# index-tts/index-tts

Hardware: AMD Instinct MI355X
Metric: audio-seconds/sec (RTF) IndexTTS-2.5, 64-utt batch @1/2/4/8 MI355X (higher is better)
Workload: dtype bf16 (GPT GEMM operands / KV cache; f32 accumulate, residual stream, norms: the reference's own GPU mode) + fp32x3 (flow matching: f32 activations / weights / accumulation, GEMM and attention products on the bf16 matrix pipe with every f32 operand carried exactly as three bf16 planes = 24 significan

## Files before the change

### indextts_amd/csrc/capi_s2mel.hip

```cpp
#include <math.h>
#include <stdlib.h>
#include <string.h>
#include <algorithm>
#include <map>
#include <string>
#include <vector>

#include "../../include/indextts_hip.h"
#include "gpt_kernels.h"
#include "s2mel_kernels.h"

static bool s2_fused(int precision, bool opt_fused) {
    if (precision == PREC_F32X3) return true;
    return (precision == PREC_BF16 || precision == PREC_F32) && opt_fused;
}

struct S2Layer {
    void *w_qkv = 0, *w_o = 0, *w_13 = 0, *w_2 = 0, *w_skip_a = 0, *w_skip_b = 0;
    float *g_attn = 0, *g_ffn = 0, *b_skip = 0;
};
struct S2Wn {
    void *w_in = 0, *w_rs = 0;
    float *b_in = 0, *b_rs = 0;
};

struct itts_s2mel {
    itts_s2mel_config cfg;
    int I = 0, Kx = 0;
    std::map<std::string, std::pair<std::vector<float>, std::vector<int64_t>>> host;
    std::vector<S2Layer> layers;
    std::vector<S2Wn> wn;
    float* g_norm = 0;
    void *w_x = 0, *w_sl_a = 0, *w_sl_b = 0, *w_c1 = 0, *w_rp = 0, *w_fl = 0, *w_c2 = 0;
    float *b_sl = 0, *b_c1 = 0, *b_rp = 0, *b_fl = 0, *b_c2 = 0;
    std::vector<void*> owned;
    bool finalized = false;
    bool opt_fused = true;
// ... 287 lines not shown
        if (!rc) rc = f.pack_kn(Fin::cols_kn(*wc2, C, W, 0, W), W, W, C, &h->w_c2);
        if (!rc) rc = f.vec(bc2, &h->b_c2);
    }
    for (int i = 0; i < L && rc == ITTS_OK; ++i) {
        const std::string a = P + "wavenet.in_layers." + std::to_string(i) + ".conv.conv.", b = P + "wavenet.res_skip_layers." + std::to_string(i) + ".conv.conv.";
        const int ro = i < L - 1 ? 2 * W : W;
        NEED(wi, a + "weight", 2 * W, W, k);
        NEED(bi, a + "bias", 2 * W);
        NEED(wr, b + "weight", ro, W, 1);
        NEED(br, b + "bias", ro);
        if (!wi || !bi || !wr || !br) continue;
        std::vector<float> kn((size_t)k * W * 2 * W);
        for (int n = 0; n < 2 * W; ++n)
            for (int cc = 0; cc < W; ++cc)
                for (int j = 0; j < k; ++j) kn[((size_t)j * W + cc) * 2 * W + n] = (*wi)[((size_t)n * W + cc) * k + j];
        rc = f.pack_kn(f.pair_tiles(kn, k * W, 2 * W), k * W, k * W, 2 * W, &h->wn[i].w_in);
        if (!rc) rc = f.vec(bi, &h->wn[i].b_in);
        if (!rc) rc = f.pack_kn(Fin::cols_kn(*wr, ro, W, 0, W), W, W, ro, &h->wn[i].w_rs);
        if (!rc) rc = f.vec(br, &h->wn[i].b_rs);
    }
#undef NEED
    if (rc) return rc;
    if (!f.missing.empty()) { itts_set_error("s2mel_finalize: missing or mis-shaped tensors: %s", f.missing.c_str()); return ITTS_ERR_STATE; }
    h->host.clear();
    h->finalized = true;
    return ITTS_OK;
}

extern "C" int itts_s2mel_mods_per_step(const itts_s2mel* h) {
    if (!h) return 0;
    const itts_s2mel_config& c = h->cfg;
    return c.depth * 4 * c.hidden_dim + 2 * c.hidden_dim + c.wavenet_layers * 2 * c.wavenet_hidden + 2 * c.wavenet_hidden;
}

static size_t s_a256(size_t x) { return (x + 255) & ~(size_t)255; }

struct S2Ws {
    float *X, *X2, *BIG, *WX, *OUT, *RP, *D;
    char *HB, *QA, *AO, *FC, *COL, *XA, *SK, *KC, *VC, *WXA, *ZR, *HBP;
    size_t hbp_stride;
    size_t sk_stride, total;
};

static S2Ws s2_carve(const itts_s2mel* h, char* base, int n_tok, int n_seq, int t_pad) {
    const itts_s2mel_config& c = h->cfg;
    const size_t N = (size_t)n_tok, H = c.hidden_dim, I = h->I, W = c.wavenet_hidden, C = c.in_channels, Kx = h->Kx;
    const size_t esz = c.precision == PREC_BF16 ? 2 : 4;
    const size_t big = std::max(std::max(3 * H, 2 * I), 2 * W);
    const size_t hw = std::max(H, W), fw = std::max(I, W);
    S2Ws w;
    size_t off = 0;
    auto take = [&](size_t bytes) { char* p = base ? base + off : nullptr; off += s_a256(bytes); return p; };
    w.X = (float*)take(N * H * 4);
    w.X2 = (float*)take(N * H * 4);
    w.BIG = (float*)take(N * big * 4);
    w.WX = (float*)take(N * W * 4);
    w.OUT = (float*)take(N * W * 4);
    w.RP = (float*)take(N * W * 4);
    w.D = (float*)take(N * C * 4);
    w.HB = take(N * hw * esz);
    w.QA = take(N * H * esz);
    w.AO = take(N * H * esz);
    w.FC = take(N * fw * esz);
    w.COL = take(N * (size_t)c.wavenet_kernel * W * esz);
    w.XA = take(N * Kx * esz);
    w.sk_stride = s_a256(N * H * esz);
    w.SK = take(w.sk_stride * (size_t)(c.depth / 2));
    w.WXA = take(N * W * esz);
    w.hbp_stride = (N * H + 127) / 128 * 128;
    w.HBP = take(c.precision == PREC_F32X3 ? w.hbp_stride * 6 : 0);
    const size_t kv = (size_t)n_seq * c.num_heads * t_pad * 64 * (c.precision == PREC_F32X3 ? 6 : esz);
    w.ZR = take(256);
    w.KC = take(kv);
    w.VC = take(kv);
    w.total = off + 256;
    return w;
}

extern "C" size_t itts_s2mel_workspace_bytes(const itts_s2mel* h, int n_tok, int n_seq, int t_max) {
    if (!h || n_tok <= 0 || n_seq <= 0 || t_max <= 0) return 0;
    return s2_carve(h, nullptr, n_tok, n_seq, (t_max + 63) / 64 * 64).total;
}

// ... 117 lines not shown
    const float* m_gc = m_norm + 2 * H;
    const float* m_fl = m_gc + (size_t)c.wavenet_layers * 2 * W;
    const SeqTab& tt = tail ? *tail : tab;
    const void* XAt = w.XA;
    if (tail) {
        if ((rc = launch_cast_pad(x_src, w.QA, tail->n_tok, src_rows, C, Kx, prec, st, tail_src))) return rc;
        XAt = w.QA;
    }
    const int NT = tt.n_tok;
    if ((rc = launch_ada_rmsnorm(X, h->g_norm, m_norm, w.HB, NT, H, c.norm_eps, prec, st, tail && !prune_last ? tail_src : nullptr))) return rc;
    S2_TRACE("final ada_rmsnorm -> HB", w.HB, (size_t)NT * H * esz);
    if ((rc = s2_gemm(h, w.HB, H, h->w_sl_a, h->b_sl, X2, H, NT, H, H, EPI_STORE_F32, st))) return rc;
    if ((rc = s2_gemm(h, XAt, Kx, h->w_sl_b, nullptr, X2, H, NT, H, Kx, EPI_RESIDUAL, st, fused ? w.HB : nullptr))) return rc;
    if (!fused && (rc = launch_cast_pad(X2, w.HB, NT, NT, H, H, prec, st))) return rc;
    S2_TRACE("skip_linear -> X2", X2, (size_t)NT * H * 4);
    if ((rc = s2_gemm(h, w.HB, H, h->w_c1, h->b_c1, w.WX, W, NT, W, H, EPI_STORE_F32, st, fused ? w.WXA : nullptr))) return rc;
    S2_TRACE("conv1 -> WX", w.WX, (size_t)NT * W * 4);
    if ((rc = s2_gemm(h, w.HB, H, h->w_rp, h->b_rp, w.RP, W, NT, W, H, EPI_STORE_F32, st))) return rc;
    int dil = 1;
    for (int i = 0; i < c.wavenet_layers; ++i) {
        const S2Wn& Wn = h->wn[i];
        const int last = i == c.wavenet_layers - 1;
        if (!fused && (rc = launch_im2col_reflect(w.WX, w.COL, tt, W, c.wavenet_kernel, dil, prec, st))) return rc;
        const int ro = last ? W : 2 * W;
        if (fused) {
            GemmArgs g{};
            g.A = w.WXA; g.lda = W; g.Wp = Wn.w_in; g.bias = Wn.b_in; g.M = NT; g.N = 2 * W; g.K = c.wavenet_kernel * W;
            g.nsplit = 1; g.epi = EPI_GATE; g.out_act = w.FC; g.gvec = m_gc + (size_t)i * 2 * W; g.D = W;
            g.conv_taps = c.wavenet_kernel; g.conv_dil = dil; g.conv_W = W; g.tok_seq = tt.tok_seq; g.tok_t = tt.tok_t;
            g.seq_start = tt.seq_start; g.seq_T = tt.seq_T; g.zero_row = w.ZR;
            if ((rc = s2_launch_gemm(h, g, st))) return rc;
            GemmArgs r{};
            r.A = w.FC; r.lda = W; r.Wp = Wn.w_rs; r.bias = Wn.b_rs; r.M = NT; r.N = ro; r.K = W; r.nsplit = 1; r.epi = EPI_WN_RS;
            r.out_f32 = w.WX; r.out2 = w.OUT; r.D = W; r.wn_first = i == 0; r.wn_last = last; r.out_act2 = last ? nullptr : w.WXA;
            r.tok_seq = tt.tok_seq; r.tok_t = tt.tok_t; r.seq_len = tt.seq_len;
            S2_TRACE("wavenet in_layer + gate -> FC", w.FC, (size_t)NT * W * esz);
            if ((rc = s2_launch_gemm(h, r, st))) return rc;
            S2_TRACE("wavenet res_skip -> WX", w.WX, (size_t)NT * W * 4);
            S2_TRACE("wavenet res_skip -> OUT", w.OUT, (size_t)NT * W * 4);
        } else {
            if ((rc = s2_gemm(h, w.COL, c.wavenet_kernel * W, Wn.w_in, Wn.b_in, w.BIG, 2 * W, NT, 2 * W, c.wavenet_kernel * W, EPI_STORE_F32, st))) return rc;
            if ((rc = launch_wn_gate(w.BIG, m_gc + (size_t)i * 2 * W, w.FC, NT, W, prec, st))) return rc;
            if ((rc = s2_gemm(h, w.FC, W, Wn.w_rs, Wn.b_rs, w.BIG, ro, NT, ro, W, EPI_STORE_F32, st))) return rc;
            if ((rc = launch_wn_update(w.BIG, w.WX, w.OUT, tt, W, i == 0, last, st))) return rc;
        }
        dil *= c.wavenet_dilation_rate;
    }
    if ((rc = launch_final_ln_mod(w.OUT, w.RP, m_fl, w.HB, tt, W, prec, st))) return rc;
    if ((rc = s2_gemm(h, w.HB, W, h->w_fl, h->b_fl, w.BIG, W, NT, W, W, EPI_STORE_F32, st, fused ? w.FC : nullptr))) return rc;
// ... 163 lines not shown
```

### indextts_amd/csrc/common.h

```cpp
#pragma once
#include <hip/hip_runtime.h>
#include <stdint.h>
#include <stdio.h>
#include <string.h>

#define ITTS_OK 0
#define ITTS_ERR_ARG 1
#define ITTS_ERR_HIP 2
#define ITTS_ERR_STATE 3
#define ITTS_ERR_NOMEM 4

#define HIP_TRY(expr)                                                                         \
    do {                                                                                      \
        hipError_t _e = (expr);                                                               \
        if (_e != hipSuccess) {                                                               \
            itts_set_error("%s:%d %s -> %s", __FILE__, __LINE__, #expr, hipGetErrorString(_e)); \
            return ITTS_ERR_HIP;                                                              \
        }                                                                                     \
    } while (0)

void itts_set_error(const char* fmt, ...);

enum { OPT_DECODE_FUSE_LN, OPT_DECODE_GEMM, OPT_DECODE_ROT, OPT_DECODE_WNT, OPT_DECODE_NT, OPT_PREFILL_GEMM, OPT_TILE256, OPT_F32_TILE,
       OPT_X3_PRODUCTS, OPT_X3_SCHED, OPT_X3_ATTN, OPT_SAMPLE_RADIX, OPT_GPT_COMPACT, OPT_ATTN_WAVES, OPT_S2MEL_FUSED, OPT_FA_QS,
       OPT_F32_ATTN_SCALAR, OPT_FA32_QS, OPT_AA_ACT, OPT_CONV_BM, OPT_H3_KERNEL, OPT_DECODE_LN_NT, OPT_X3_APLANES, OPT_X3_PIN, OPT_PREFILL_ATTN, OPT_VOC_ACT_PLANES, OPT_X3_WAVES, OPT_S2MEL_PRUNE_LAST, OPT_X3_ATTN_SKIP, OPT_COUNT };
int itts_opt(int id);
unsigned itts_opt_epoch();

typedef float f32x4 __attribute__((ext_vector_type(4)));
typedef float f32x16 __attribute__((ext_vector_type(16)));
typedef short bf16x8 __attribute__((ext_vector_type(8)));
typedef unsigned short u16;

static inline int ceil_div(int a, int b) { return (a + b - 1) / b; }

struct ItDevGuard {
    int prev = -1;
    bool switched = false;
    explicit ItDevGuard(int dev) {
        if (dev < 0) return;
// ... 55 lines not shown
```

### indextts_amd/csrc/gemm_tile.h

```cpp
#pragma once
#include "gpt_kernels.h"
#include <type_traits>

typedef __bf16 bf16x8_t __attribute__((ext_vector_type(8)));
typedef unsigned int v4u __attribute__((ext_vector_type(4)));

__device__ __forceinline__ float gelu_new_f(float x) {
    const float c = 0.7978845608028654f;
    return 0.5f * x * (1.0f + tanhf(c * (x + 0.044715f * x * x * x)));
}

#define PF_BM 128
#define PF_BN 128
#define PF_BK 64
#define PF_GM 8
#define PF_LDS 67584
#ifndef PF_SCHED
#define PF_SCHED 1
#endif

__device__ __forceinline__ uint32_t pf_pack2(float a, float b) { return (uint32_t)f32_to_bf16(a) | ((uint32_t)f32_to_bf16(b) << 16); }

template <int EPI>
__device__ __forceinline__ void pf_epilogue(const GemmArgs& a, int mbase, int nbase, int lane, f32x4 v) {
// ... 173 lines not shown
            f32x4 o;
            if constexpr (EPI == EPI_SWIGLU) {
#pragma unroll
                for (int q = 0; q < 4; ++q) o[q] = va[q] * pf_sigmoid_t<F32>(va[q]) * vb[q];
            } else {
#pragma unroll
                for (int q = 0; q < 4; ++q) o[q] = pf_tanh_t<F32>(va[q] + b1[q]) * pf_sigmoid_t<F32>(vb[q] + b2[q]);
            }
            pf_store_act4<F32>(a.out_act, (size_t)m * half + n, o);
        } else {
            f32x4 v = *(const f32x4*)(ct + row * 128 + (ca ^ sw));
#pragma unroll
            for (int q = 0; q < 4; ++q) v[q] += b1[q];
            if constexpr (EPI == EPI_STORE_F32) {
                *(f32x4*)(a.out_f32 + (size_t)m * a.ldo + n) = v;
                if (a.out_act2) pf_store_act4<F32>(a.out_act2, (size_t)m * a.ldo + n, v);
            } else if constexpr (EPI == EPI_RESIDUAL) {
                f32x4* o = (f32x4*)(a.out_f32 + (size_t)m * a.ldo + n);
                const f32x4 old = *o;
#pragma unroll
                for (int q = 0; q < 4; ++q) v[q] += old[q];
                *o = v;
                if (a.out_act2) pf_store_act4<F32>(a.out_act2, (size_t)m * a.ldo + n, v);
            } else if constexpr (EPI == EPI_RESIDUAL_SRC) {
                const f32x4 old = *(const f32x4*)(a.res_src + (size_t)meta[row] * a.ldo + n);
#pragma unroll
                for (int q = 0; q < 4; ++q) v[q] += old[q];
                *(f32x4*)(a.out_f32 + (size_t)m * a.ldo + n) = v;
                if (a.out_act2) pf_store_act4<F32>(a.out_act2, (size_t)m * a.ldo + n, v);
            } else if constexpr (EPI == EPI_GELU_ACT) {
#pragma unroll
// ... 5 lines not shown
                if (a.wn_last || n >= a.D) {
                    f32x4* o = (f32x4*)(a.out2 + (size_t)m * a.D + (a.wn_last ? n : n - a.D));
                    if (!a.wn_first) {
                        const f32x4 old = *o;
#pragma unroll
                        for (int q = 0; q < 4; ++q) v[q] += old[q];
                    }
                    *o = v;
                } else {
                    const float mask = (float)meta[row];
                    f32x4* o = (f32x4*)(a.out_f32 + (size_t)m * a.D + n);
                    const f32x4 old = *o;
#pragma unroll
                    for (int q = 0; q < 4; ++q) v[q] = (old[q] + v[q]) * mask;
                    *o = v;
                    if (a.out_act2) pf_store_act4<F32>(a.out_act2, (size_t)m * a.D + n, v);
                }
            } else if constexpr (EPI == EPI_QKV) {
                if (which == 0) {
                    *(f32x4*)(a.qbuf + (size_t)m * a.D + c) = v;
                } else {
                    const int b = m / a.S, si = m - b * a.S;
                    const size_t pb = (size_t)b * (a.seq_mul > 1 ? a.seq_mul : 1);
                    const int pos = *a.pos_ptr + si - (a.pos_shift ? a.pos_shift[pb] : 0);
                    const size_t o = ((pb * a.H + hd) * a.Tmax + pos) * 64 + d;
                    if constexpr (F32) *(f32x4*)((float*)(which == 1 ? a.kcache : a.vcache) + o) = v;
                    else *(v2u_t*)((u16*)(which == 1 ? a.kcache : a.vcache) + o) =
                        v2u_t{(uint32_t)f32_to_bf16(v[0]) | ((uint32_t)f32_to_bf16(v[1]) << 16), (uint32_t)f32_to_bf16(v[2]) | ((uint32_t)f32_to_bf16(v[3]) << 16)};
                }
            } else {
                const int sq = meta[row], t = meta[ROWS + row];
// ... 105 lines not shown
```

### indextts_amd/csrc/gemm_x3.hip

```cpp
#include "gemm_tile.h"

#define X3_LDS PF_LDS
#define X3_LDS_ONE (96 * 1024)

typedef const __attribute__((address_space(1))) char* pf_gptr_t;
__device__ __forceinline__ pf_gptr_t pf_uni(const char* p) {
    const uint64_t u = (uint64_t)p;
    const uint32_t lo = __builtin_amdgcn_readfirstlane((uint32_t)u), hi = __builtin_amdgcn_readfirstlane((uint32_t)(u >> 32));
    return (pf_gptr_t)(((uint64_t)hi << 32) | lo);
}

__device__ __forceinline__ void x3_split8(const f32x4 p0, const f32x4 p1, v4u& H, v4u& M, v4u& L) {
    const float x[8] = {p0[0], p0[1], p0[2], p0[3], p1[0], p1[1], p1[2], p1[3]};
#pragma unroll
    for (int i = 0; i < 4; ++i) {
        const float a = x[2 * i], b = x[2 * i + 1];
        const uint32_t h = pf_cvt2(a, b);
        const float ra = a - __uint_as_float(h << 16), rb = b - __uint_as_float(h & 0xffff0000u);
        const uint32_t m = pf_cvt2(ra, rb);
        const float sa = ra - __uint_as_float(m << 16), sb = rb - __uint_as_float(m & 0xffff0000u);
        H[i] = h; M[i] = m; L[i] = pf_cvt2(sa, sb);
    }
}

template <int EPI, bool CONV = false, int NPROD = 8, bool SCHED = true, bool APL = false>
__global__ __launch_bounds__(256, 2) void gemm_x3_kernel(GemmArgs a) {
    extern __shared__ __attribute__((aligned(16))) char pf_sm[];
    const int lane = threadIdx.x & 63, w = __builtin_amdgcn_readfirstlane(threadIdx.x >> 6);
    const int wr = w >> 1, wc = w & 1;
    const int n_mt = (a.M + PF_BM - 1) / PF_BM, n_nt = (a.N + PF_BN - 1) / PF_BN;
    const int total = n_mt * n_nt, per = (total + 7) >> 3;
    const int t = (int)(blockIdx.x & 7) * per + (int)(blockIdx.x >> 3);
    if (t >= total) return;
    const int g0 = t / (PF_GM * n_nt), first_m = g0 * PF_GM;
    const int gm = (n_mt - first_m) < PF_GM ? (n_mt - first_m) : PF_GM;
    const int r = t - g0 * PF_GM * n_nt;
    const int bn = r / gm, bm = first_m + (r - bn * gm);
// ... 50 lines not shown
    auto issue_a = [&](int kt, int buf) {
        char* base = pf_sm + buf * STAGE;
        if constexpr (APL) {
#pragma unroll
            for (int i = 0; i < 6; ++i)
                __builtin_amdgcn_global_load_lds((const __attribute__((address_space(1))) void*)(pf_uni(abase + (size_t)(i >> 1) * a.a_planes * 2 + (size_t)kt * 64) + aoff[i]),
                                                 (__attribute__((address_space(3))) void*)(base + (i >> 1) * 8192 + (w + 4 * (i & 1)) * 1024), 16, 0, 0);
            return;
        }
        int tap = 0, rem = kt;
        if constexpr (CONV) { tap = kt / cv_kpt; rem = kt - tap * cv_kpt; }
#pragma unroll
        for (int i = 0; i < 4; ++i) {
            const char* ap = asrc[i] + (size_t)kt * 128;
            if constexpr (CONV) {
                const int maxpad = cv_left;
                const int Tv = cv_T[i] <= maxpad ? maxpad + 1 : cv_T[i];
                int p = cv_t[i] + tap * a.conv_dil - cv_left;
                p = p < 0 ? -p : p;
                p = p >= Tv ? 2 * (Tv - 1) - p : p;
                const bool ok = p >= 0 && p < cv_T[i];
                ap = ok ? cv_base[i] + ((size_t)p * a.lda + (size_t)rem * 32) * 4 : cv_zero[i];
            }
            if constexpr (CONV)
                __builtin_amdgcn_global_load_lds((const __attribute__((address_space(1))) void*)ap,
                                                 (__attribute__((address_space(3))) void*)(base + (w * 4 + i) * 1024), 16, 0, 0);
            else
                __builtin_amdgcn_global_load_lds((const __attribute__((address_space(1))) void*)(pf_uni(abase + (size_t)kt * 128) + aoff[i]),
                                                 (__attribute__((address_space(3))) void*)(base + (w * 4 + i) * 1024), 16, 0, 0);
        }
    };
    auto load_w = [&](int kt, v4u (&bw)[4][3]) {
#pragma unroll
        for (int nt = 0; nt < 4; ++nt)
#pragma unroll
            for (int p = 0; p < 3; ++p) bw[nt][p] = *(const __attribute__((address_space(1))) v4u*)(pf_uni(wbase[nt] + (size_t)kt * 3072) + lane16 + p * 1024);
// ... 149 lines not shown
    const uint32_t lane16 = lane * 16;
#pragma unroll
    for (int i = 0; i < 3; ++i) {
        const int q = w + 8 * i;
        int ntile = nt0 + q / 3;
        ntile = ntile < ntiles ? ntile : ntiles - 1;
        wdma[i] = (const char*)a.Wp + (size_t)ntile * nk * 3072 + (q % 3) * 1024;
    }
    auto issue = [&](int kt, int buf) {
        char* base = pf_sm + buf * X3W8_STAGE;
        int tap = 0, rem = kt;
        if constexpr (CONV) { tap = kt / cv_kpt; rem = kt - tap * cv_kpt; }
#pragma unroll
        for (int i = 0; i < 2; ++i) {
            if constexpr (CONV) {
                const int maxpad = cv_left;
                const int Tv = cv_T[i] <= maxpad ? maxpad + 1 : cv_T[i];
                int p = cv_t[i] + tap * a.conv_dil - cv_left;
                p = p < 0 ? -p : p;
                p = p >= Tv ? 2 * (Tv - 1) - p : p;
                const bool ok = p >= 0 && p < cv_T[i];
                const char* ap = ok ? cv_base[i] + ((size_t)p * a.lda + (size_t)rem * 32) * 4 : cv_zero[i];
                __builtin_amdgcn_global_load_lds((const __attribute__((address_space(1))) void*)ap,
                                                 (__attribute__((address_space(3))) void*)(base + (w * 2 + i) * 1024), 16, 0, 0);
            } else {
                (void)asrc;
                __builtin_amdgcn_global_load_lds((const __attribute__((address_space(1))) void*)(pf_uni(abase + (size_t)kt * 128) + aoff[i]),
                                                 (__attribute__((address_space(3))) void*)(base + (w * 2 + i) * 1024), 16, 0, 0);
            }
        }
#pragma unroll
        for (int i = 0; i < 3; ++i)
            __builtin_amdgcn_global_load_lds((const __attribute__((address_space(1))) void*)(pf_uni(wdma[i] + (size_t)kt * 3072) + lane16),
                                             (__attribute__((address_space(3))) void*)(base + 16384 + (w + 8 * i) * 1024), 16, 0, 0);
    };

// ... 66 lines not shown
        __syncthreads();
        pf_store_vt<128, 512, true>(a, ct, m0, nt0 * 16, threadIdx.x);
        return;
    }
#pragma unroll
    for (int mt = 0; mt < 2; ++mt)
#pragma unroll
        for (int nt = 0; nt < 4; ++nt)
#pragma unroll
            for (int rr = 0; rr < 4; ++rr)
                ct[(wr * 32 + mt * 16 + g * 4 + rr) * 128 + ((wc * 64 + nt * 16 + c16) ^ (g << 4))] = acc[mt][nt][rr];
    int* meta = (int*)(pf_sm + 65536);
    pf_stage_meta<EPI, 128>(a, meta, m0, threadIdx.x);
    __syncthreads();
    pf_store_tile<EPI, 128, 512, true>(a, ct, meta, m0, nt0 * 16, threadIdx.x);
}

template <int EPI, bool CONV = false>
static int launch_gemm_x3_e(const GemmArgs& a, hipStream_t st) {
    const int n_mt = ceil_div(a.M, PF_BM), n_nt = ceil_div(a.N, PF_BN);
    const int per = ceil_div(n_mt * n_nt, 8);
    const int nprod = itts_opt(OPT_X3_PRODUCTS) == 6 ? 6 : 8;
    const bool sched = itts_opt(OPT_X3_SCHED) != 0;
    static ItPerDevice<bool> attr_set_pd;
    bool& attr_set = attr_set_pd.cur();
    if (!attr_set) {
        HIP_TRY(hipFuncSetAttribute((const void*)gemm_x3_kernel<EPI, CONV, 8, true>, hipFuncAttributeMaxDynamicSharedMemorySize, X3_LDS_ONE));
        HIP_TRY(hipFuncSetAttribute((const void*)gemm_x3_kernel<EPI, CONV, 6, true>, hipFuncAttributeMaxDynamicSharedMemorySize, X3_LDS_ONE));
        HIP_TRY(hipFuncSetAttribute((const void*)gemm_x3_kernel<EPI, CONV, 8, false>, hipFuncAttributeMaxDynamicSharedMemorySize, X3_LDS_ONE));
        HIP_TRY(hipFuncSetAttribute((const void*)gemm_x3_kernel<EPI, CONV, 6, false>, hipFuncAttributeMaxDynamicSharedMemorySize, X3_LDS_ONE));
// ... 75 lines not shown
```

### indextts_amd/csrc/gpt_kernels.h

```cpp
#pragma once
#include "common.h"

enum { PREC_F32 = 0, PREC_BF16 = 1,
       PREC_F32X3 = 2 };

struct LnArgs {
    float* x;
    const float* partial;
    int nsplit;
    const float* bias_prev;
    const float* g1; const float* b1;
    const float* g2; const float* b2;
    void* out;
    int out_f32;
    int rows, D;
    int in_row_mul, in_row_add;
    float eps;
};
int launch_ln(const LnArgs& a, int prec, hipStream_t st);

enum { EPI_STORE_F32 = 0, EPI_GELU_ACT = 1, EPI_PARTIAL = 2, EPI_RESIDUAL = 3, EPI_QKV = 4,
       EPI_SWIGLU = 5,
       EPI_GATE = 6,
       EPI_QKV_ROPE = 7,
// ... 14 lines not shown
    const int* pos_shift;
    size_t a_planes;
    int kb_slice;
    int dma_rot;
    const float* ln_x; float* ln_x_out; const float* ln_partial; const float* ln_bias_prev; const float* ln_g; const float* ln_b; float ln_eps;
    const int* tok_seq; const int* tok_t; const int* seq_len; const float* rope; const float* gvec;
    float* out2; int wn_first, wn_last;
    int conv_taps, conv_dil, conv_W;
    const int* seq_start; const int* seq_T; const void* zero_row;
    void* out_act2;
    int seq_mul;
    const int* seq_map;
    size_t kv_planes;
    const float* res_src;
    const int* res_map;
};
int launch_gemm(const GemmArgs& a, int prec, bool prefill, hipStream_t st);
int launch_gemm_x3(const GemmArgs& a, hipStream_t st);
int gemm_x3_occupancy(int* blocks);
bool gemm_decode_ln_ok(int M, int K, int epi);
int launch_gemm_decode_ln(const GemmArgs& a, hipStream_t st);
int gemm_tile_occupancy(int prec, int* blocks);

enum GemmPath {
    GP_NONE = -1,
    GP_BF16_TILE128, GP_BF16_TILE128_NOVEC, GP_BF16_TILE256, GP_BF16_TILE256X128, GP_BF16_REG_PREFILL,
    GP_BF16_SLAB_MT1, GP_BF16_SLAB_MT2, GP_BF16_SLAB_MT4_NT1, GP_BF16_SLAB_MT4_NT2, GP_BF16_SLAB_MT4_NT4,
    GP_BF16_REG_DECODE_MT1, GP_BF16_REG_DECODE_MT2, GP_BF16_REG_DECODE_MT4,
    GP_F32_TILE, GP_F32_REG_PREFILL, GP_F32_REG_DECODE_MT1, GP_F32_REG_DECODE_MT2, GP_F32_REG_DECODE_MT4,
    GP_X3_4W_P6, GP_X3_4W_P8, GP_X3_4W_APLANES, GP_X3_8W,
    GP_BF16_LN_DECODE_4W, GP_BF16_LN_DECODE_WIDE_NT2, GP_BF16_LN_DECODE_WIDE_NT4,
    GP_COUNT
};
void gemm_note_path(int path);
// ... 189 lines not shown
```

### indextts_amd/csrc/options.hip

```cpp
#include <atomic>
#include <stdlib.h>
#include <string.h>

#include "../../include/indextts_hip.h"
#include "common.h"

namespace {
struct OptDef {
    const char* name;
    int def, lo, hi;
    const char* doc;
    const char* allowed = nullptr;
};
const OptDef kDefs[OPT_COUNT] = {
    {"decode_fuse_ln", 1, 0, 2, "GPT decode: LayerNorm (+ split-K reduce, bias, residual) inside the consuming GEMM -- 1: steps of 1-8 rows (measured faster), 2: up to 16 rows (measured slower above 8, kept for the A/B record), 0: separate ln_kernel launches; bitwise equal"},
    {"decode_gemm", 1, 0, 1, "bf16 decode GEMMs on the LDS-DMA slab kernel (0: register-path gemm_kernel; bitwise equal)"},
    {"decode_rot", 1, 0, 1, "per-block rotation of the slab DMA issue order in the decode GEMM (same bytes, same LDS image)"},
    {"decode_wnt", 0, 0, 1, "non-temporal policy on the decode GEMM's weight stream"},
    {"decode_nt", 0, 0, 4, "force the n-tiles per block of the 64-row decode GEMM (0: smallest that fits one round of blocks)", "0,1,2,4"},
    {"prefill_gemm", 1, 0, 1, "bf16 prefill GEMMs on the LDS-DMA tile kernels (0: register-path gemm_kernel; bitwise equal)"},
    {"tile256", -1, -1, 2, "bf16 tile GEMM: -1 pick by shape, 0 always 128x128, 1 always 256x256, 2 always 256x128 (bitwise equal)"},
    {"f32_tile", 1, 0, 1, "f32 GEMMs with plain epilogues on the f32-MFMA tile kernel (0: register-path kernel; bitwise equal)"},
    {"x3_products", 6, 6, 8, "plane products per f32 product of the fp32x3 GEMMs and attention: 6 (hh, hm, mh, hl, lh, mm; drops m*l and l*m, 2^-24 |ab| each: measured error vs f64 <= the native f32-MFMA kernels' on every benchmarked shape) or 8 (every term down to 2^-24 |ab|; two blocks per CU like the default since the packed-RoPE fix -- option x3_pin = 1 restores round 4's one-block pin as a diagnostic)", "6,8"},
    {"x3_sched", 1, 0, 1, "fp32x3 GEMM: interleave the operand split with the MFMAs (0: split as a burst; bitwise equal)"},
// ... 4 lines not shown
    {"s2mel_fused", 1, 0, 2, "s2mel: fused GEMM epilogues, sampled when a handle is created -- 1: fused, 0: separate element-wise kernels (2: round 4's spelling of 'the bf16 wqkv epilogue fused too'; the same as 1 since the RoPE fix of round 5)"},
    {"fa_qs", 0, 0, 4, "bf16 flash attention: query sub-tiles per wave (0: pick by shape)", "0,1,2,4"},
    {"f32_attn_scalar", 0, 0, 1, "f32 s2mel attention on the one-wave-per-query reference kernel (the A/B path of the f32 flash kernel)"},
    {"fa32_qs", 2, 1, 2, "f32 flash attention: query sub-tiles per wave"},
    {"aa_act", 2, 0, 2, "anti-aliased activation kernel variant (2: swizzled LDS tiles)"},
    {"conv_bm", 0, 0, 128, "force the co-tile height of conv_mfma_kernel (0: pick by channel count)", "0,32,64,96,128"},
    {"h3_kernel", 1, 0, 1, "f16x3 vocoder conv: 1 window kernel, 0 two-stage kernel"},
    {"decode_ln_nt", 2, 2, 4, "LayerNorm-fused decode GEMM at 5-16 rows (weights on waves 0-3, LayerNorm on waves 4-7): n-tiles per block, 2 or 4 (bitwise equal)", "2,4"},
    {"x3_aplanes", 0, 0, 1, "fp32x3 s2mel: the adaptive-RMSNorm outputs as three bf16 planes in fragment order, wqkv / w1|w3 GEMMs without an operand split (bitwise equal)"},
    {"x3_pin", 0, 0, 1, "fp32x3 GEMM: 1 pins the variants that are not the default one (8 products, burst split) to one block per CU -- round 4's workaround for their run-to-run differences, kept as a diagnostic; not needed since the RoPE fix of round 5 (DESIGN.md section 9)"},
    {"prefill_attn", -1, -1, 1, "attention of S > 1 passes (prefill, latent pass): -1 causal MFMA kernel in the bf16 mode, canonical-stream kernel in the f32 parity mode; 0 canonical-stream kernel (one block per query) always; 1 MFMA kernel in both precisions"},
    {"voc_act_planes", 1, 0, 1, "vocoder, bf16x3 conv mode: the anti-aliased activation in front of an x3 conv writes the conv's three operand planes itself (aa_act_planes_kernel); 0: f32 activation + split pass (bit-identical planes)"},
    {"x3_waves", 8, 4, 8, "fp32x3 GEMM: waves per 128 x 128 block -- 8 (4 x 2, wave tile 32 x 64, weights through LDS: four waves per SIMD at two blocks per CU; 64-utterance solve 314.7 vs 323.0 ms per Euler step, profiles/r06k) or 4 (2 x 2, wave tile 64 x 64, weights in registers: round 5's kernel); bitwise equal", "4,8"},
    {"s2mel_prune_last", 1, 0, 1, "fp32x3 s2mel solve with a tail layout: the LAST DiT layer's attention runs the queries of the tail rows only (keys / values: every frame) and writes the tail layout, its wo / FFN norm / w1|w3 / w2 stages run on the tail rows (residual gathered by a row map in the wo epilogue); the x_in GEMM reads its residual from const_in instead of a copy of it; 0: every row, copy first (bitwise equal)"},
    {"x3_attn_skip", 1, 0, 1, "fp32x3 flash attention: a last key tile with <= 32 valid keys skips the MFMAs of its fully masked half, and a wave whose 32 queries are all out of range only stages its share of K / V^T (0: full tiles, every wave computes; bitwise equal)"},
};
std::atomic<int> g_val[OPT_COUNT];
std::atomic<unsigned> g_epoch{1};
std::atomic<bool> g_init{false};

void ensure_init() {
    if (g_init.load(std::memory_order_acquire)) return;
    static std::atomic_flag once = ATOMIC_FLAG_INIT;
    if (!once.test_and_set()) {
        for (int i = 0; i < OPT_COUNT; ++i) g_val[i].store(kDefs[i].def, std::memory_order_relaxed);
        g_init.store(true, std::memory_order_release);
    } else {
        while (!g_init.load(std::memory_order_acquire)) {}
    }
}
// ... 54 lines not shown
```

Measured before the change: 142.3.

## Add windowed fp32x3 WaveNet in_layer conv kernel reusing staged plane windows across taps

Adds a dedicated kernel for the WaveNet in_layer dilated convs in the fp32x3 path. The conv1 and res_skip epilogues now write the activation directly as three bf16 planes. The kernel stages one 256-row window plus halo per 32-channel chunk once, and every tap reads it at a row offset, so the activation is no longer re-gathered per tap and the split happens once per element. Weights are pre-packed per tap into three planes at finalize. Accumulation order changes to chunk-outer, tap-inner, so the low bits differ from the previous path. The new path is on by default and only taken when every layer's kernel size and dilation fit the halo.

```diff
diff --git a/indextts_amd/csrc/capi_s2mel.hip b/indextts_amd/csrc/capi_s2mel.hip
--- a/indextts_amd/csrc/capi_s2mel.hip
+++ b/indextts_amd/csrc/capi_s2mel.hip
@@ -21,6 +21,7 @@
 };
 struct S2Wn {
     void *w_in = 0, *w_rs = 0;
+    void* w_in_win = 0;
     float *b_in = 0, *b_rs = 0;
 };
 
@@ -338,7 +339,13 @@
         for (int n = 0; n < 2 * W; ++n)
             for (int cc = 0; cc < W; ++cc)
                 for (int j = 0; j < k; ++j) kn[((size_t)j * W + cc) * 2 * W + n] = (*wi)[((size_t)n * W + cc) * k + j];
-        rc = f.pack_kn(f.pair_tiles(kn, k * W, 2 * W), k * W, k * W, 2 * W, &h->wn[i].w_in);
+        const std::vector<float> knp = f.pair_tiles(kn, k * W, 2 * W);
+        rc = f.pack_kn(knp, k * W, k * W, 2 * W, &h->wn[i].w_in);
+        if (!rc && c.precision == PREC_F32X3 && wn_window_x3_ok(W, k, 1)) {
+            std::vector<char> pk(wn_window_x3_packed_bytes(k * W, 2 * W));
+            rc = wn_window_x3_pack(knp.data(), k, W, 2 * W, pk.data());
+            if (!rc) rc = s2_upload(h, pk.data(), pk.size(), &h->wn[i].w_in_win);
+        }
         if (!rc) rc = f.vec(bi, &h->wn[i].b_in);
         if (!rc) rc = f.pack_kn(Fin::cols_kn(*wr, ro, W, 0, W), W, W, ro, &h->wn[i].w_rs);
         if (!rc) rc = f.vec(br, &h->wn[i].b_rs);
@@ -364,7 +371,12 @@
     char *HB, *QA, *AO, *FC, *COL, *XA, *SK, *KC, *VC, *WXA, *ZR, *HBP;
     size_t hbp_stride;
     size_t sk_stride, total;
+    size_t wxa_stride;
 };
+
+static bool s2_wn_window_opt(const itts_s2mel* h) {
+    return h->cfg.precision == PREC_F32X3 && itts_opt(OPT_S2MEL_WN_WINDOW) != 0 && itts_opt(OPT_X3_PRODUCTS) == 6;
+}
 
 static S2Ws s2_carve(const itts_s2mel* h, char* base, int n_tok, int n_seq, int t_pad) {
     const itts_s2mel_config& c = h->cfg;
@@ -390,7 +402,8 @@
     w.XA = take(N * Kx * esz);
     w.sk_stride = s_a256(N * H * esz);
     w.SK = take(w.sk_stride * (size_t)(c.depth / 2));
-    w.WXA = take(N * W * esz);
+    w.wxa_stride = s2_wn_window_opt(h) ? N * W : 0;
+    w.WXA = take(N * W * (w.wxa_stride ? 6 : esz));
     w.hbp_stride = (N * H + 127) / 128 * 128;
     w.HBP = take(c.precision == PREC_F32X3 ? w.hbp_stride * 6 : 0);
     const size_t kv = (size_t)n_seq * c.num_heads * t_pad * 64 * (c.precision == PREC_F32X3 ? 6 : esz);
@@ -538,7 +551,16 @@
     if ((rc = s2_gemm(h, XAt, Kx, h->w_sl_b, nullptr, X2, H, NT, H, Kx, EPI_RESIDUAL, st, fused ? w.HB : nullptr))) return rc;
     if (!fused && (rc = launch_cast_pad(X2, w.HB, NT, NT, H, H, prec, st))) return rc;
     S2_TRACE("skip_linear -> X2", X2, (size_t)NT * H * 4);
-    if ((rc = s2_gemm(h, w.HB, H, h->w_c1, h->b_c1, w.WX, W, NT, W, H, EPI_STORE_F32, st, fused ? w.WXA : nullptr))) return rc;
+    bool wn_win = w.wxa_stride != 0 && s2_wn_window_opt(h);
+    for (int i = 0, d = 1; i < c.wavenet_layers && wn_win; ++i, d *= c.wavenet_dilation_rate)
+        wn_win = h->wn[i].w_in_win != nullptr && wn_window_x3_ok(W, c.wavenet_kernel, d);
+    {
+        GemmArgs g{};
+        g.A = w.HB; g.lda = H; g.Wp = h->w_c1; g.bias = h->b_c1; g.M = NT; g.N = W; g.K = H; g.nsplit = 1; g.epi = EPI_STORE_F32; g.out_f32 = w.WX; g.ldo = W; g.D = W;
+        g.out_act2 = fused ? w.WXA : nullptr;
+        g.act2_planes = wn_win ? w.wxa_stride : 0;
+        if ((rc = s2_launch_gemm(h, g, st))) return rc;
+    }
     S2_TRACE("conv1 -> WX", w.WX, (size_t)NT * W * 4);
     if ((rc = s2_gemm(h, w.HB, H, h->w_rp, h->b_rp, w.RP, W, NT, W, H, EPI_STORE_F32, st))) return rc;
     int dil = 1;
@@ -553,10 +575,15 @@
             g.nsplit = 1; g.epi = EPI_GATE; g.out_act = w.FC; g.gvec = m_gc + (size_t)i * 2 * W; g.D = W;
             g.conv_taps = c.wavenet_kernel; g.conv_dil = dil; g.conv_W = W; g.tok_seq = tt.tok_seq; g.tok_t = tt.tok_t;
             g.seq_start = tt.seq_start; g.seq_T = tt.seq_T; g.zero_row = w.ZR;
-            if ((rc = s2_launch_gemm(h, g, st))) return rc;
+            if (wn_win) {
+                g.Wp = Wn.w_in_win; g.a_planes = w.wxa_stride;
+                S2Prof ps(h, st, S2_GEMM, 2.0 * g.M * (double)g.N * g.K);
+                if ((rc = launch_wn_window_x3(g, st))) return rc;
+            } else if ((rc = s2_launch_gemm(h, g, st))) return rc;
             GemmArgs r{};
             r.A = w.FC; r.lda = W; r.Wp = Wn.w_rs; r.bias = Wn.b_rs; r.M = NT; r.N = ro; r.K = W; r.nsplit = 1; r.epi = EPI_WN_RS;
             r.out_f32 = w.WX; r.out2 = w.OUT; r.D = W; r.wn_first = i == 0; r.wn_last = last; r.out_act2 = last ? nullptr : w.WXA;
+            r.act2_planes = wn_win ? w.wxa_stride : 0;
             r.tok_seq = tt.tok_seq; r.tok_t = tt.tok_t; r.seq_len = tt.seq_len;
             S2_TRACE("wavenet in_layer + gate -> FC", w.FC, (size_t)NT * W * esz);
             if ((rc = s2_launch_gemm(h, r, st))) return rc;
diff --git a/indextts_amd/csrc/common.h b/indextts_amd/csrc/common.h
--- a/indextts_amd/csrc/common.h
+++ b/indextts_amd/csrc/common.h
@@ -23,7 +23,7 @@
 
 enum { OPT_DECODE_FUSE_LN, OPT_DECODE_GEMM, OPT_DECODE_ROT, OPT_DECODE_WNT, OPT_DECODE_NT, OPT_PREFILL_GEMM, OPT_TILE256, OPT_F32_TILE,
        OPT_X3_PRODUCTS, OPT_X3_SCHED, OPT_X3_ATTN, OPT_SAMPLE_RADIX, OPT_GPT_COMPACT, OPT_ATTN_WAVES, OPT_S2MEL_FUSED, OPT_FA_QS,
-       OPT_F32_ATTN_SCALAR, OPT_FA32_QS, OPT_AA_ACT, OPT_CONV_BM, OPT_H3_KERNEL, OPT_DECODE_LN_NT, OPT_X3_APLANES, OPT_X3_PIN, OPT_PREFILL_ATTN, OPT_VOC_ACT_PLANES, OPT_X3_WAVES, OPT_S2MEL_PRUNE_LAST, OPT_X3_ATTN_SKIP, OPT_COUNT };
+       OPT_F32_ATTN_SCALAR, OPT_FA32_QS, OPT_AA_ACT, OPT_CONV_BM, OPT_H3_KERNEL, OPT_DECODE_LN_NT, OPT_X3_APLANES, OPT_X3_PIN, OPT_PREFILL_ATTN, OPT_VOC_ACT_PLANES, OPT_X3_WAVES, OPT_S2MEL_PRUNE_LAST, OPT_X3_ATTN_SKIP, OPT_S2MEL_WN_WINDOW, OPT_COUNT };
 int itts_opt(int id);
 unsigned itts_opt_epoch();
 
diff --git a/indextts_amd/csrc/gemm_tile.h b/indextts_amd/csrc/gemm_tile.h
--- a/indextts_amd/csrc/gemm_tile.h
+++ b/indextts_amd/csrc/gemm_tile.h
@@ -211,7 +211,8 @@
             for (int q = 0; q < 4; ++q) v[q] += b1[q];
             if constexpr (EPI == EPI_STORE_F32) {
                 *(f32x4*)(a.out_f32 + (size_t)m * a.ldo + n) = v;
-                if (a.out_act2) pf_store_act4<F32>(a.out_act2, (size_t)m * a.ldo + n, v);
+                if (F32 && a.act2_planes) pf_store_planes4(a.out_act2, a.act2_planes, (size_t)m * a.ldo + n, v);
+                else if (a.out_act2) pf_store_act4<F32>(a.out_act2, (size_t)m * a.ldo + n, v);
             } else if constexpr (EPI == EPI_RESIDUAL) {
                 f32x4* o = (f32x4*)(a.out_f32 + (size_t)m * a.ldo + n);
                 const f32x4 old = *o;
@@ -247,7 +248,8 @@
 #pragma unroll
                     for (int q = 0; q < 4; ++q) v[q] = (old[q] + v[q]) * mask;
                     *o = v;
-                    if (a.out_act2) pf_store_act4<F32>(a.out_act2, (size_t)m * a.D + n, v);
+                    if (F32 && a.act2_planes) pf_store_planes4(a.out_act2, a.act2_planes, (size_t)m * a.D + n, v);
+                    else if (a.out_act2) pf_store_act4<F32>(a.out_act2, (size_t)m * a.D + n, v);
                 }
             } else if constexpr (EPI == EPI_QKV) {
                 if (which == 0) {
diff --git a/indextts_amd/csrc/gemm_x3.hip b/indextts_amd/csrc/gemm_x3.hip
--- a/indextts_amd/csrc/gemm_x3.hip
+++ b/indextts_amd/csrc/gemm_x3.hip
@@ -1,3 +1,5 @@
+#include <string.h>
+
 #include "gemm_tile.h"
 
 #define X3_LDS PF_LDS
@@ -21,6 +23,14 @@
         const float sa = ra - __uint_as_float(m << 16), sb = rb - __uint_as_float(m & 0xffff0000u);
         H[i] = h; M[i] = m; L[i] = pf_cvt2(sa, sb);
     }
+}
+
+__device__ __forceinline__ bool x3_conv_src(int t, int T, int tap, int dil, int left, int& p) {
+    const int Tv = T <= left ? left + 1 : T;
+    p = t + tap * dil - left;
+    p = p < 0 ? -p : p;
+    p = p >= Tv ? 2 * (Tv - 1) - p : p;
+    return p >= 0 && p < T;
 }
 
 template <int EPI, bool CONV = false, int NPROD = 8, bool SCHED = true, bool APL = false>
@@ -101,12 +111,8 @@
         for (int i = 0; i < 4; ++i) {
             const char* ap = asrc[i] + (size_t)kt * 128;
             if constexpr (CONV) {
-                const int maxpad = cv_left;
-                const int Tv = cv_T[i] <= maxpad ? maxpad + 1 : cv_T[i];
-                int p = cv_t[i] + tap * a.conv_dil - cv_left;
-                p = p < 0 ? -p : p;
-                p = p >= Tv ? 2 * (Tv - 1) - p : p;
-                const bool ok = p >= 0 && p < cv_T[i];
+                int p;
+                const bool ok = x3_conv_src(cv_t[i], cv_T[i], tap, a.conv_dil, cv_left, p);
                 ap = ok ? cv_base[i] + ((size_t)p * a.lda + (size_t)rem * 32) * 4 : cv_zero[i];
             }
             if constexpr (CONV)
@@ -286,12 +292,8 @@
 #pragma unroll
         for (int i = 0; i < 2; ++i) {
             if constexpr (CONV) {
-                const int maxpad = cv_left;
-                const int Tv = cv_T[i] <= maxpad ? maxpad + 1 : cv_T[i];
-                int p = cv_t[i] + tap * a.conv_dil - cv_left;
-                p = p < 0 ? -p : p;
-                p = p >= Tv ? 2 * (Tv - 1) - p : p;
-                const bool ok = p >= 0 && p < cv_T[i];
+                int p;
+                const bool ok = x3_conv_src(cv_t[i], cv_T[i], tap, a.conv_dil, cv_left, p);
                 const char* ap = ok ? cv_base[i] + ((size_t)p * a.lda + (size_t)rem * 32) * 4 : cv_zero[i];
                 __builtin_amdgcn_global_load_lds((const __attribute__((address_space(1))) void*)ap,
                                                  (__attribute__((address_space(3))) void*)(base + (w * 2 + i) * 1024), 16, 0, 0);
@@ -388,6 +390,239 @@
     pf_stage_meta<EPI, 128>(a, meta, m0, threadIdx.x);
     __syncthreads();
     pf_store_tile<EPI, 128, 512, true>(a, ct, meta, m0, nt0 * 16, threadIdx.x);
+}
+
+#define WNW_BM 256
+#define WNW_HALO 8
+#define WNW_NCH ((WNW_BM + 2 * WNW_HALO) / 16)
+#define WNW_ACH (WNW_NCH + 1)
+#define WNW_ZROW (WNW_NCH * 16)
+#define WNW_ABUF (3 * WNW_ACH * 1024)
+#define WNW_NWT 8
+#define WNW_WST (3 * WNW_NWT * 1024)
+#define WNW_LDS (2 * WNW_ABUF + 2 * WNW_WST)
+#define WNW_MT 4
+#define WNW_NT 4
+
+template <int N>
+__device__ __forceinline__ void wnw_wait_vm() { asm volatile("s_waitcnt vmcnt(%0)" ::"n"(N) : "memory"); }
+
+template <int NH>
+__global__ __launch_bounds__(512) __attribute__((amdgpu_waves_per_eu(2, 2))) void wn_window_x3_kernel(GemmArgs a, int n_mt, int n_co) {
+    extern __shared__ __attribute__((aligned(16))) char pf_sm[];
+    const int lane = threadIdx.x & 63, w = __builtin_amdgcn_readfirstlane(threadIdx.x >> 6);
+    const int wr = w >> 1, wc = w & 1;
+    const int L = blockIdx.x;
+    const int xcd = L & 7, slot = L >> 3;
+    const int tile = (slot / n_co) * 8 + xcd;
+    if (tile >= n_mt) return;
+    const int m0 = tile * WNW_BM;
+    const int nt0 = (slot % n_co) * (WNW_NWT * NH);
+    const int k = a.conv_taps, dil = a.conv_dil;
+    const int nkc = a.conv_W >> 5, G = k * nkc * NH;
+    const int left = ((k - 1) * dil) / 2;
+
+    const int row16 = lane & 15, kg = lane >> 4;
+    int r_t[WNW_MT], r_T[WNW_MT], r_w0[WNW_MT];
+#pragma unroll
+    for (int mt = 0; mt < WNW_MT; ++mt) {
+        int m = m0 + (wr * WNW_MT + mt) * 16 + row16;
+        m = m < a.M ? m : a.M - 1;
+        const int sq = a.tok_seq[m];
+        r_t[mt] = a.tok_t[m];
+        r_T[mt] = a.seq_T[sq];
+        r_w0[mt] = a.seq_start[sq] - (m0 - WNW_HALO);
+    }
+    if (threadIdx.x < 384) {
+        const int q = threadIdx.x >> 6;
+        *(v4u*)(pf_sm + (q / 3) * WNW_ABUF + ((q % 3) * WNW_ACH + WNW_NCH) * 1024 + lane * 16) = v4u{0u, 0u, 0u, 0u};
+    }
+    __syncthreads();
+
+    const size_t plane = a.a_planes * 2;
+    const char* zr = (const char*)a.zero_row;
+    const int my_ach = (WNW_NCH - w + 7) >> 3;
+    const char* asrc[3];
+    bool aok[3];
+#pragma unroll
+    for (int i = 0; i < 3; ++i) {
+        const int m = m0 - WNW_HALO + (w + 8 * i) * 16 + row16;
+        aok[i] = m >= 0 && m < a.M;
+        asrc[i] = (const char*)a.A + ((size_t)(aok[i] ? m : 0) * a.lda + kg * 8) * 2;
+    }
+    auto issue_a = [&](int kc_, int buf) {
+        char* base = pf_sm + buf * WNW_ABUF;
+#pragma unroll
+        for (int i = 0; i < 3; ++i) {
+            const int c = w + 8 * i;
+            if (c < WNW_NCH) {
+#pragma unroll
+                for (int pl = 0; pl < 3; ++pl)
+                    __builtin_amdgcn_global_load_lds((const __attribute__((address_space(1))) void*)(aok[i] ? asrc[i] + pl * plane + (size_t)kc_ * 64 : zr),
+                                                     (__attribute__((address_space(3))) void*)(base + (pl * WNW_ACH + c) * 1024), 16, 0, 0);
+            }
+        }
+    };
+    const char* wsrc = (const char*)a.Wp + ((size_t)(nt0 + w) * nkc * k) * 3072 + lane * 16;
+    auto issue_w = [&](int g) {
+        const int kc_ = g / (k * NH), r_ = g - kc_ * k * NH;
+        const int h_ = r_ / k, j_ = r_ - h_ * k;
+        const char* src = wsrc + ((size_t)h_ * WNW_NWT * nkc * k + (size_t)kc_ * k + j_) * 3072;
+        char* base = pf_sm + 2 * WNW_ABUF + (g & 1) * WNW_WST;
+#pragma unroll
+        for (int pl = 0; pl < 3; ++pl)
+            __builtin_amdgcn_global_load_lds((const __attribute__((address_space(1))) void*)(src + pl * 1024),
+                                             (__attribute__((address_space(3))) void*)(base + (pl * WNW_NWT + w) * 1024), 16, 0, 0);
+    };
+
+    f32x4 acc[NH][WNW_MT][WNW_NT];
+#pragma unroll
+    for (int h = 0; h < NH; ++h)
+#pragma unroll
+        for (int i = 0; i < WNW_MT; ++i)
+#pragma unroll
+            for (int jn = 0; jn < WNW_NT; ++jn) acc[h][i][jn] = f32x4{0.f, 0.f, 0.f, 0.f};
+
+    const int b_off = wc * WNW_NT * 1024 + lane * 16;
+    auto a_off = [&](int mt, int j) {
+        int p;
+        const bool ok = x3_conv_src(r_t[mt], r_T[mt], j, dil, left, p);
+        int rr = r_w0[mt] + p;
+        rr = rr < 0 ? 0 : rr;
+        rr = ok && rr < WNW_ZROW ? rr : WNW_ZROW;
+        return (rr >> 4) * 1024 + kg * 256 + (rr & 15) * 16;
+    };
+
+    issue_a(0, 0);
+    issue_w(0);
+    bool a_recent = false;
+    v4u afc[WNW_MT][3];
+    auto ktile = [&](int g, int kc, int kc_n, int j_n, f32x4 (&ac)[WNW_MT][WNW_NT], bool first_of_chunk) {
+        if (a_recent) { if (my_ach == 3) wnw_wait_vm<9>(); else wnw_wait_vm<6>(); } else wnw_wait_vm<0>();
+        __builtin_amdgcn_s_barrier();
+        asm volatile("" ::: "memory");
+        if (g + 1 < G) issue_w(g + 1);
+        a_recent = false;
+        if (first_of_chunk && kc + 1 < nkc) { issue_a(kc + 1, (kc + 1) & 1); a_recent = true; }
+        const char* wbase = pf_sm + 2 * WNW_ABUF + (g & 1) * WNW_WST;
+        v4u bf[WNW_NT][3];
+#pragma unroll
+        for (int nt = 0; nt < WNW_NT; ++nt)
+#pragma unroll
+            for (int pl = 0; pl < 3; ++pl) bf[nt][pl] = *(const v4u*)(wbase + pl * WNW_NWT * 1024 + b_off + nt * 1024);
+        if (g == 0) {
+#pragma unroll
+            for (int mt = 0; mt < WNW_MT; ++mt) {
+                const char* ap = pf_sm + a_off(mt, 0);
+#pragma unroll
+                for (int pl = 0; pl < 3; ++pl) afc[mt][pl] = *(const v4u*)(ap + pl * WNW_ACH * 1024);
+            }
+        }
+        const char* abase_n = pf_sm + (kc_n & 1) * WNW_ABUF;
+        const bool more = g + 1 < G;
+#pragma unroll
+        for (int mt = 0; mt < WNW_MT; ++mt) {
+            constexpr int PA[6] = {2, 0, 1, 1, 0, 0};
+            constexpr int PB[6] = {0, 2, 1, 0, 1, 0};
+#pragma unroll
+            for (int q = 0; q < 6; ++q)
+#pragma unroll
+                for (int nt = 0; nt < WNW_NT; ++nt)
+                    ac[mt][nt] = __builtin_amdgcn_mfma_f32_16x16x32_bf16(__builtin_bit_cast(bf16x8_t, afc[mt][PA[q]]),
+                                                                         __builtin_bit_cast(bf16x8_t, bf[nt][PB[q]]), ac[mt][nt], 0, 0, 0);
+            if (more) {
+                const char* ap = abase_n + a_off(mt, j_n);
+#pragma unroll
+                for (int pl = 0; pl < 3; ++pl) afc[mt][pl] = *(const v4u*)(ap + pl * WNW_ACH * 1024);
+            }
+        }
+    };
+    {
+        int g = 0;
+        for (int kc = 0; kc < nkc; ++kc) {
+#pragma unroll
+            for (int h = 0; h < NH; ++h)
+                for (int j = 0; j < k; ++j, ++g) {
+                    int j_n = j + 1, kc_n = kc;
+                    if (j_n == k) { j_n = 0; if (h == NH - 1) kc_n = kc + 1; }
+                    ktile(g, kc, kc_n, j_n, acc[h], h == 0 && j == 0);
+                }
+        }
+    }
+    float* ct = (float*)pf_sm;
+    const int g4 = lane >> 4, c16 = lane & 15;
+#pragma unroll
+    for (int h = 0; h < NH; ++h) {
+        __syncthreads();
+#pragma unroll
+        for (int mt = 0; mt < WNW_MT; ++mt)
+#pragma unroll
+            for (int nt = 0; nt < WNW_NT; ++nt)
+#pragma unroll
+                for (int rr = 0; rr < 4; ++rr)
+                    ct[(wr * 64 + mt * 16 + g4 * 4 + rr) * 128 + ((wc * 64 + nt * 16 + c16) ^ (g4 << 4))] = acc[h][mt][nt][rr];
+        __syncthreads();
+        pf_store_tile<EPI_GATE, WNW_BM, 512, true>(a, ct, nullptr, m0, (nt0 + h * WNW_NWT) * 16, threadIdx.x);
+    }
+}
+
+bool wn_window_x3_ok(int W, int taps, int dil) {
+    return W >= 32 && W % 32 == 0 && (2 * W) % (WNW_NWT * 16) == 0 && (taps & 1) && taps >= 3 && dil >= 1 && (taps - 1) * dil <= 2 * WNW_HALO;
+}
+
+size_t wn_window_x3_packed_bytes(int K, int N) { return (size_t)(N / 16) * (K / 32) * 3072; }
+
+static uint16_t wnw_bf16_rne(float f) {
+    uint32_t u;
+    memcpy(&u, &f, 4);
+    u += 0x7fffu + ((u >> 16) & 1u);
+    return (uint16_t)(u >> 16);
+}
+static float wnw_bf16_f(uint16_t h) { const uint32_t u = (uint32_t)h << 16; float f; memcpy(&f, &u, 4); return f; }
+
+int wn_window_x3_pack(const float* kn, int taps, int W, int N, void* out) {
+    if (!kn || !out || taps < 1 || W < 32 || W % 32 || N < 16 || N % 16) { itts_set_error("wn_window_x3_pack: need W %% 32 == 0 and N %% 16 == 0 (taps=%d W=%d N=%d)", taps, W, N); return ITTS_ERR_ARG; }
+    const int nkc = W / 32;
+    uint16_t* o = (uint16_t*)out;
+    for (int nt = 0; nt < N / 16; ++nt)
+        for (int kc = 0; kc < nkc; ++kc)
+            for (int j = 0; j < taps; ++j) {
+                uint16_t* rec = o + (((size_t)nt * nkc + kc) * taps + j) * 1536;
+                for (int ln = 0; ln < 64; ++ln)
+                    for (int e = 0; e < 8; ++e) {
+                        const float f = kn[((size_t)j * W + kc * 32 + (ln >> 4) * 8 + e) * N + nt * 16 + (ln & 15)];
+                        if (!(f - f == 0.f)) { itts_set_error("wn_window_x3_pack: weight %g is not finite", (double)f); return ITTS_ERR_ARG; }
+                        const uint16_t h = wnw_bf16_rne(f);
+                        const float r = f - wnw_bf16_f(h);
+                        const uint16_t m = wnw_bf16_rne(r);
+                        rec[ln * 8 + e] = h; rec[512 + ln * 8 + e] = m; rec[1024 + ln * 8 + e] = wnw_bf16_rne(r - wnw_bf16_f(m));
+                    }
+            }
+    return ITTS_OK;
+}
+
+int launch_wn_window_x3(const GemmArgs& a, hipStream_t st) {
+    if (a.M <= 0) return ITTS_OK;
+    if (a.epi != EPI_GATE || !wn_window_x3_ok(a.conv_W, a.conv_taps, a.conv_dil) || a.N != 2 * a.conv_W || a.K != a.conv_taps * a.conv_W || a.lda != a.conv_W ||
+        !a.a_planes || !a.A || !a.Wp || !a.gvec || !a.out_act || !a.tok_seq || !a.tok_t || !a.seq_start || !a.seq_T || !a.zero_row || (((uintptr_t)a.A | (uintptr_t)a.Wp) & 15) ||
+        (a.a_planes & 7)) {
+        itts_set_error("wn_window (f32x3): need the gate epilogue in tap mode on plane operands, W %% 64 == 0, an odd kernel size and (k - 1) * dil <= %d (W=%d k=%d dil=%d)",
+                       2 * WNW_HALO, a.conv_W, a.conv_taps, a.conv_dil);
+        return ITTS_ERR_ARG;
+    }
+    const int n_mt = ceil_div(a.M, WNW_BM);
+    const int n_co = a.N / (WNW_NWT * 16);
+    const long long nblocks = (long long)ceil_div(n_mt, 8) * 8 * n_co;
+    if (nblocks > 2147483647ll) { itts_set_error("wn_window (f32x3): grid too large"); return ITTS_ERR_ARG; }
+    static ItPerDevice<bool> attr_set_pd;
+    bool& attr_set = attr_set_pd.cur();
+    if (!attr_set) {
+        HIP_TRY(hipFuncSetAttribute((const void*)wn_window_x3_kernel<1>, hipFuncAttributeMaxDynamicSharedMemorySize, WNW_LDS));
+        attr_set = true;
+    }
+    hipLaunchKernelGGL(wn_window_x3_kernel<1>, dim3((unsigned)nblocks), dim3(512), WNW_LDS, st, a, n_mt, n_co);
+    HIP_TRY(hipGetLastError());
+    return ITTS_OK;
 }
 
 template <int EPI, bool CONV = false>
diff --git a/indextts_amd/csrc/gpt_kernels.h b/indextts_amd/csrc/gpt_kernels.h
--- a/indextts_amd/csrc/gpt_kernels.h
+++ b/indextts_amd/csrc/gpt_kernels.h
@@ -52,10 +52,15 @@
     size_t kv_planes;
     const float* res_src;
     const int* res_map;
+    size_t act2_planes;
 };
 int launch_gemm(const GemmArgs& a, int prec, bool prefill, hipStream_t st);
 int launch_gemm_x3(const GemmArgs& a, hipStream_t st);
 int gemm_x3_occupancy(int* blocks);
+bool wn_window_x3_ok(int W, int taps, int dil);
+size_t wn_window_x3_packed_bytes(int K, int N);
+int wn_window_x3_pack(const float* kn, int taps, int W, int N, void* out);
+int launch_wn_window_x3(const GemmArgs& a, hipStream_t st);
 bool gemm_decode_ln_ok(int M, int K, int epi);
 int launch_gemm_decode_ln(const GemmArgs& a, hipStream_t st);
 int gemm_tile_occupancy(int prec, int* blocks);
diff --git a/indextts_amd/csrc/options.hip b/indextts_amd/csrc/options.hip
--- a/indextts_amd/csrc/options.hip
+++ b/indextts_amd/csrc/options.hip
@@ -42,6 +42,7 @@
     {"x3_waves", 8, 4, 8, "fp32x3 GEMM: waves per 128 x 128 block -- 8 (4 x 2, wave tile 32 x 64, weights through LDS: four waves per SIMD at two blocks per CU; 64-utterance solve 314.7 vs 323.0 ms per Euler step, profiles/r06k) or 4 (2 x 2, wave tile 64 x 64, weights in registers: round 5's kernel); bitwise equal", "4,8"},
     {"s2mel_prune_last", 1, 0, 1, "fp32x3 s2mel solve with a tail layout: the LAST DiT layer's attention runs the queries of the tail rows only (keys / values: every frame) and writes the tail layout, its wo / FFN norm / w1|w3 / w2 stages run on the tail rows (residual gathered by a row map in the wo epilogue); the x_in GEMM reads its residual from const_in instead of a copy of it; 0: every row, copy first (bitwise equal)"},
     {"x3_attn_skip", 1, 0, 1, "fp32x3 flash attention: a last key tile with <= 32 valid keys skips the MFMAs of its fully masked half, and a wave whose 32 queries are all out of range only stages its share of K / V^T (0: full tiles, every wave computes; bitwise equal)"},
+    {"s2mel_wn_window", 1, 0, 1, "fp32x3 s2mel (fused, 6 plane products): the WaveNet in_layer convs on wn_window_x3_kernel -- their operand arrives as three row-major bf16 planes written by the conv1 / res_skip epilogues, the plane windows of a 32-channel chunk are staged once and every tap reads them at a row offset (chunk-outer, tap-inner accumulation: the low bits differ from 0); taken when every layer fits (kernel size odd, (k - 1) * dilation <= 16); 0: f32 shadow + the tap-mode GEMM"},
 };
 std::atomic<int> g_val[OPT_COUNT];
 std::atomic<unsigned> g_epoch{1};
```

New measurement: 143.4 (median of 6 runs). Within noise of the previous version (+0.8%).
